# heyblackC/DFMIR

Hardware: AMD Instinct MI355X
Metric: train-step image-pairs/sec (fwd+bwd): 2D 256x256 bs=16 and 3D 160^3 bs=1 (higher is better)
Workload: dtype f32 (fp16x2-split MFMA, fp32 accumulate)

## Files before the change

### dfmir_amd/_lib.py

```python
import ctypes
import os
from ctypes import c_float, c_int, c_longlong, c_void_p, POINTER, Structure

_HERE = os.path.dirname(os.path.abspath(__file__))
LIB_PATH = os.environ.get("DFMIR_HIP_LIB") or os.path.join(_HERE, "libdfmir_hip.so")


class DfConvGeom(Structure):
    _fields_ = [(n, c_int) for n in (
        "N", "Cin", "Cout", "Di", "Hi", "Wi", "Do", "Ho", "Wo", "KD", "KH", "KW",
        "stride", "dil", "pd", "ph", "pw", "pad_mode", "act")] + [("slope", c_float)]


P = c_void_p
_GP = POINTER(DfConvGeom)
_SIGS = {
    "dfmir_abi_version": [],
    "dfmir_set_option": [ctypes.c_char_p, ctypes.c_char_p],
    "dfmir_get_option": [ctypes.c_char_p, ctypes.c_char_p, c_int],
    "dfmir_conv_fwd": [_GP, P, P, P, P, P],
    "dfmir_conv_wgrad": [_GP, P, P, P, P],
    "dfmir_bias_grad": [P, P, c_int, c_int, c_longlong, P],
    "dfmir_weight_pack": [P, P, c_int, c_int, c_int, c_int, P],
    "dfmir_weight_pack_floats": [c_int, c_int, c_int],
    "dfmir_weight_pack_batch": [P, c_int, P, c_int, P],
    "dfmir_conv3x3_res_ok": [_GP],
    "dfmir_conv3x3_fwd_scaled_res": [_GP, P, P, c_int, P, P, P, P, c_int, P, P],
    "dfmir_conv3x3_reflect_ring_ok": [_GP],
    "dfmir_conv3x3_reflect_ring_len": [_GP],
    "dfmir_conv3x3_reflect_ring": [_GP, P, P, P, c_int, P, P, P],
    "dfmir_conv_fwd_scaled": [_GP, P, P, c_int, P, P, P, P],
    "dfmir_conv_wgrad_scaled": [_GP, P, P, c_int, P, P, c_int, P, P, P],
    "dfmir_conv_wgrad_scaled_ch": [_GP, P, P, c_int, P, P, c_int, P, P, P, P],
    "dfmir_instnorm_bwd_pmax_ok": [c_longlong],
    "dfmir_instnorm_bwd_pmax": [P, P, P, P, P, c_int, c_longlong, c_int, P, P, c_int, P, P],
    "dfmir_patch_gather_bwd_gp": [P, P, P, c_int, c_int, c_longlong, c_int, c_int, P, P, P],
    "dfmir_patch_gather_bwd_any": [P, P, P, c_int, c_int, c_longlong, c_int, c_int, P, P, P],
    "dfmir_absmax": [P, c_longlong, P, P],
    "dfmir_conv3d_split_ok": [_GP],
    "dfmir_conv3d_split_ws_floats": [c_int, c_int],
    "dfmir_conv3d_split_fwd": [_GP, P, P, c_int, P, P, P, P, P, P],
    "dfmir_conv3d_split_fwd_sub": [_GP, P, P, c_int, P, P, P, P, P, c_int, P],
    "dfmir_conv3d_split_fwd_actgrad": [_GP, P, P, c_int, P, P, P, P, P, c_int, P, c_float, P],
    "dfmir_conv3d_up_ok": [c_int] * 6,
    "dfmir_conv3d_wsplit_batch": [P, c_int, P],
    "dfmir_conv3d_split_is_pair": [c_int],
    "dfmir_conv3d_march_ok": [_GP],
    "dfmir_conv3d_march_fwd": [_GP, P, P, c_int, P, P, P, P, P, c_float, P],
    "dfmir_conv3d_tiny_ok": [_GP],
    "dfmir_conv3d_tiny_fwd": [_GP, P, P, P, P, P, P, c_float, P],
    "dfmir_conv3d_s2c2_ok": [_GP],
    "dfmir_conv3d_s2c2_fwd": [_GP, P, P, P, P, P, P],
    "dfmir_conv3d_s2c2_wgrad": [_GP, P, P, P, P],
    "dfmir_conv3d_s2_ok": [_GP],
    "dfmir_conv3d_s2_fwd": [_GP, P, P, P, P, P, P],
    "dfmir_conv3d_s2_wgrad": [_GP, P, P, P, P, P],
    "dfmir_conv3d_s2_dgrad_ok": [_GP],
    "dfmir_conv3d_s2_dgrad": [_GP, P, P, P, P],
    "dfmir_conv3d_up_ws_floats": [c_int, c_int],
    "dfmir_conv3d_up_fwd": [P, P, c_int, P, c_int, P, P] + [c_int] * 6 + [P],
    "dfmir_conv3d_up_skip2_fwd": [P, P, c_int, P, P, c_int, c_int, P, P, P, P, P] + [c_int] * 7 + [c_float, P],
    "dfmir_conv3d_up_dgrad_ws_floats": [c_int, c_int],
    "dfmir_conv3d_up_dgrad": [P, P, c_int, P, c_int, P, P, P, P, c_float] + [c_int] * 6 + [P],
    "dfmir_conv3d_split_fwd_add": [_GP, P, P, c_int, P, c_int, c_int, P, P, P, P, P],
    "dfmir_conv3d_split_wgrad_ok": [_GP],
    "dfmir_conv3d_split_wgrad": [_GP, P, P, c_int, P, P, c_int, P, P],
# ... 95 lines not shown
    "dfmir_det_begin": [P, c_longlong, P, c_longlong, P, c_int, P, c_longlong, P, c_int, ctypes.c_double, P],
    "dfmir_det_end": [P, P, c_longlong, P, c_longlong, P],
    "dfmir_fill_zero": [P, c_longlong, P],
    "dfmir_sum_scaled": [P, P, c_longlong, c_float, P],
    "dfmir_fill_from_scalar": [P, P, c_longlong, c_float, P],
    "dfmir_adam_step": [P, P, P, P, c_longlong] + [c_float] * 7 + [P],
}

_lib = None


class DfmirHipError(RuntimeError):
    pass


def lib():
    global _lib
    if _lib is None:
        import torch
        if not os.path.exists(LIB_PATH):
            raise DfmirHipError(
                "libdfmir_hip.so not found at %s -- build it with `python -c 'import __graft_entry__ as g; "
                "g.build()'` or `make -C dfmir_amd/csrc` (there is no CPU fallback)" % LIB_PATH)
        h = ctypes.CDLL(LIB_PATH)
        for name, args in _SIGS.items():
            fn = getattr(h, name)
            fn.argtypes = args
            fn.restype = c_int
        h.dfmir_weight_pack_floats.restype = c_longlong
        h.dfmir_conv3d_split_ws_floats.restype = c_longlong
        h.dfmir_conv3d_up_ws_floats.restype = c_longlong
        h.dfmir_conv3d_up_dgrad_ws_floats.restype = c_longlong
        h.dfmir_conv3d_upwgrad_ws_floats.restype = c_longlong
        h.dfmir_flow_smooth_ws_floats.restype = c_longlong
        h.dfmir_nmi_ws_floats.restype = c_longlong
        h.dfmir_warp_dice_ws_floats.restype = c_longlong
        h.dfmir_label_hausdorff_ws_bytes.restype = c_longlong
        h.dfmir_dice_ws_floats.restype = c_longlong
        h.dfmir_mse_ws_floats.restype = c_longlong
        h.dfmir_warp_bwd_own_ws_floats.restype = c_longlong
        h.dfmir_resize_bwd_ws_floats.restype = c_longlong
        h.dfmir_last_error.argtypes = []
        h.dfmir_last_error.restype = ctypes.c_char_p
        _lib = h
    return _lib


def check(rc):
    if rc != 0:
        msg = lib().dfmir_last_error()
        raise DfmirHipError(msg.decode() if msg else "dfmir_hip error %d" % rc)


def set_option(name, value=None):
    check(lib().dfmir_set_option(name.encode(), None if value is None else str(value).encode()))


def get_option(name):
    buf = ctypes.create_string_buffer(256)
    n = lib().dfmir_get_option(name.encode(), buf, 256)
    return None if n < 0 else buf.value.decode()


def exported_symbols():
    return sorted(list(_SIGS.keys()) + ["dfmir_last_error"])
```

### dfmir_amd/csrc/conv.hip

```cpp
#include "conv3x3_common.h"
#include <stdlib.h>
#include <vector>

typedef float f32x16 __attribute__((ext_vector_type(16)));

struct ConvK {
  DfConvGeom g;
  int kc, nchunks;
  int Dm, Hm, Wm, ncx, ncy, ncz;
};

static inline void df_chunking(int Cin, int& kc, int& nchunks) {
  nchunks = (Cin + 15) / 16;
  int per = (Cin + nchunks - 1) / nchunks;
  kc = (per + 1) & ~1;
  if (kc < 2) kc = 2;
}

template <bool DIL2>
__device__ __forceinline__ bool conv_pixel(const ConvK& k, long long pp, long long P, int& n, int& oz, int& oy, int& ox,
                                           int& cls) {
  const DfConvGeom& g = k.g;
  cls = 0;
  if (pp >= P) { n = oz = oy = ox = 0; return false; }
// ... 611 lines not shown
    for (int r = ly; r < T * 32; r += 8) {
      const int t = r >> 5, ci = ci0 + (r & 31), co = co0 + lx;
      float v = 0.f;
      if (ci < Cin && co < Cout) {
        const long long j = ((long long)t * Cin + ci) * Cout + co;
        v = jb.src[j];
        jb.src[j] = 0.f;
      }
      tile[lx][(r & 31) * T + t] = v;
    }
    __syncthreads();
    const int ncol = 32 * T;
    for (int e = threadIdx.x; e < 32 * ncol; e += 256) {
      const int c = e / ncol, q = e - c * ncol;
      const int co = co0 + c, ci = ci0 + q / T;
      if (co < Cout && ci < Cin) jb.dst[((long long)co * Cin + ci0) * T + q] += tile[c][q];
    }
    __syncthreads();
  }
}

bool df_conv3x3_fwd_try(const DfConvGeom* g, const float* x, const float* w_tcc, const float* bias,
                        float* y, hipStream_t st, int* rc);
bool df_conv3x3_wgrad_try(const DfConvGeom* g, const float* x, const float* dy, float* dw_tcc,
                          hipStream_t st, int* rc);
bool df_conv3x3_small_wgrad_try(const DfConvGeom* g, const float* x, const float* dy, float* dw_tcc, hipStream_t st,
                                int* rc);
bool df_conv3x3_split_fwd_try(const DfConvGeom* g, const float* x, const float* x_amax, int x_n, const float* w_packed,
                              const float* bias, const float* res, const float* ring, int ring_rl, float* y,
                              hipStream_t st, int* rc);
int df_conv3x3_split_res_ok(const DfConvGeom* g);
bool df_conv3x3_split_wgrad_try(const DfConvGeom* g, const float* x, const float* x_amax, int x_n, const float* dy,
                                const float* dy_amax, int dy_n, float* dw_tcc, float* db, hipStream_t st, int* rc,
                                const float* dy_pmax);
int df_weight_split_launch(const float* w_tcc, float* packed, int K, int M, int npart, hipStream_t st);
float* df_weight_probe_slots(float* packed, int K, int M);
int df_absmax_launch(const float* x, long long n, float* out, hipStream_t st, bool zero_first);
bool df_conv3d_fwd_try(const DfConvGeom* g, const float* x, const float* w_tcc, const float* bias, float* y,
                       hipStream_t st, int* rc);
bool df_conv3d_wgrad_try(const DfConvGeom* g, const float* x, const float* dy, float* dw_tcc, hipStream_t st,
                         int* rc);
static bool use_generic_only() {
  static DfOptInt o{"DFMIR_CONV_GENERIC", 0};
  return o.get() == 1;
}

static int check_geom(const DfConvGeom* g) {
  if (!g) return -1;
  if (g->N <= 0 || g->Cin <= 0 || g->Cout <= 0) return -1;
  if (g->Di <= 0 || g->Hi <= 0 || g->Wi <= 0 || g->Do <= 0 || g->Ho <= 0 || g->Wo <= 0) return -1;
  if (g->KD <= 0 || g->KH <= 0 || g->KW <= 0 || g->KD > 15 || g->KH > 15 || g->KW > 15) return -1;
  if (g->stride < 1 || g->dil < 1) return -1;
  if (g->pad_mode != 0 && g->pad_mode != 1) return -1;
  if (g->pad_mode == 1 && g->dil != 1) return -1;
  return 0;
}

static int conv_fwd_impl(const DfConvGeom* g, const float* x, const float* x_amax, int x_n, const float* w_tcc,
                         const float* bias, float* y, void* stream);
extern "C" int dfmir_conv_fwd(const DfConvGeom* g, const float* x, const float* w_tcc,
                              const float* bias, float* y, void* stream) {
  return conv_fwd_impl(g, x, nullptr, 0, w_tcc, bias, y, stream);
}
extern "C" int dfmir_conv_fwd_scaled(const DfConvGeom* g, const float* x, const float* x_amax, int x_amax_n,
                                     const float* w_tcc, const float* bias, float* y, void* stream) {
  return conv_fwd_impl(g, x, x_amax, x_amax_n, w_tcc, bias, y, stream);
}
// ... 82 lines not shown
      } else {
        dim3 grid((unsigned)((Ps + 255) / 256), 1);
        if (g->Cout > 32) conv_mfma_k<1, 4, 2, 2, true><<<grid, 256, 0, st>>>(xs, w_tcc, bias, ys, k);
        else conv_mfma_k<1, 4, 1, 2, true><<<grid, 256, 0, st>>>(xs, w_tcc, bias, ys, k);
      }
    } else if (small_p && g->Cout <= 64) {
      dim3 grid((unsigned)((Ps + 63) / 64), (unsigned)((g->Cout + 63) / 64));
      conv_mfma_k<2, 2, 1, 1><<<grid, 256, 0, st>>>(xs, w_tcc, bias, ys, k);
    } else if (g->Cout > 64) {
      const long long big = ((Ps + 127) / 128) * ((g->Cout + 127) / 128);
      static DfOptInt big_o{"DFMIR_GEMM_BIG_MIN", 256};
  const int big_min = big_o.get();
      if (big < big_min) {
        dim3 grid((unsigned)((Ps + 63) / 64), (unsigned)((g->Cout + 63) / 64));
        conv_mfma_k<2, 2, 1, 1><<<grid, 256, 0, st>>>(xs, w_tcc, bias, ys, k);
      } else {
        dim3 grid((unsigned)((Ps + 127) / 128), (unsigned)((g->Cout + 127) / 128));
        conv_mfma_k<2, 2, 2, 2><<<grid, 256, 0, st>>>(xs, w_tcc, bias, ys, k);
      }
    } else if (g->Cout > 32) {
      dim3 grid((unsigned)((Ps + 255) / 256), 1);
      conv_mfma_k<1, 4, 2, 2><<<grid, 256, 0, st>>>(xs, w_tcc, bias, ys, k);
    } else {
      dim3 grid((unsigned)((Ps + 255) / 256), 1);
      conv_mfma_k<1, 4, 1, 2><<<grid, 256, 0, st>>>(xs, w_tcc, bias, ys, k);
    }
    DF_LAUNCH_CHECK();
  }
  return 0;
}

static int conv_wgrad_impl(const DfConvGeom* g, const float* x, const float* x_amax, int x_n, const float* dy,
                           const float* dy_amax, int dy_n, float* dw_tcc, float* db, void* stream,
                           const float* dy_pmax = nullptr);
extern "C" int dfmir_conv_wgrad_scaled_ch(const DfConvGeom* g, const float* x, const float* x_amax, int x_amax_n,
                                          const float* dy, const float* dy_amax, int dy_amax_n, const float* dy_pmax,
                                          float* dw_tcc, float* db, void* stream) {
  return conv_wgrad_impl(g, x, x_amax, x_amax_n, dy, dy_amax, dy_amax_n, dw_tcc, db, stream, dy_pmax);
}
extern "C" int dfmir_conv_wgrad(const DfConvGeom* g, const float* x, const float* dy, float* dw_tcc,
                                void* stream) {
  return conv_wgrad_impl(g, x, nullptr, 0, dy, nullptr, 0, dw_tcc, nullptr, stream);
}
extern "C" int dfmir_conv_wgrad_scaled(const DfConvGeom* g, const float* x, const float* x_amax, int x_amax_n,
                                       const float* dy, const float* dy_amax, int dy_amax_n, float* dw_tcc,
                                       float* db, void* stream) {
  return conv_wgrad_impl(g, x, x_amax, x_amax_n, dy, dy_amax, dy_amax_n, dw_tcc, db, stream);
}
static int bias_grad_launch(const float* dy, float* db, int N, int C, long long S, hipStream_t st);
static int conv_wgrad_impl(const DfConvGeom* g, const float* x, const float* x_amax, int x_n, const float* dy,
                           const float* dy_amax, int dy_n, float* dw_tcc, float* db, void* stream, const float* dy_pmax) {
  DF_ARG_CHECK(check_geom(g) == 0 && x && dy && dw_tcc);
  DF_ARG_CHECK(g->dil == 1 && g->Cin < (1 << 19));
  hipStream_t st = (hipStream_t)stream;
  if (!use_generic_only()) {
    int rc = 0;
    if (df_conv3x3_split_wgrad_try(g, x, x_amax, x_n, dy, dy_amax, dy_n, dw_tcc, db, st, &rc, dy_pmax)) return rc;
  }
  if (db) {
    const int rcb = bias_grad_launch(dy, db, g->N, g->Cout, (long long)g->Do * g->Ho * g->Wo, st);
    if (rcb) return rcb;
  }
  if (!use_generic_only()) {
    int rc = 0;
    if (df_conv3x3_wgrad_try(g, x, dy, dw_tcc, st, &rc)) return rc;
    if (df_conv3x3_small_wgrad_try(g, x, dy, dw_tcc, st, &rc)) return rc;
    if (df_conv3d_wgrad_try(g, x, dy, dw_tcc, st, &rc)) return rc;
  }
  {
    static DfOptFlag no1x1_o{"DFMIR_NO_1X1_WGRAD"};
    const long long S1 = (long long)g->Di * g->Hi * g->Wi;
    if (!use_generic_only() && !no1x1_o.get() && g->KD == 1 && g->KH == 1 && g->KW == 1 && g->stride == 1 && g->pd == 0 &&
        g->ph == 0 && g->pw == 0 && g->Do == g->Di && g->Ho == g->Hi && g->Wo == g->Wi && (S1 & 3) == 0 && S1 >= 64 &&
        ((reinterpret_cast<uintptr_t>(x) | reinterpret_cast<uintptr_t>(dy)) & 15) == 0 && g->Cin >= 8 && g->Cout >= 8) {
      const long long cpi = (S1 + 63) / 64, total = (long long)g->N * cpi;
      const unsigned ny = (unsigned)((g->Cin + 63) / 64), nz = (unsigned)((g->Cout + 63) / 64);
      long long want = 1024 / ((long long)ny * nz);
      if (want < 1) want = 1;
      long long maxs = (total + 7) / 8;
      if (maxs < 1) maxs = 1;
      if (want > maxs) want = maxs;
      const long long cpb = (total + want - 1) / want;
      const unsigned nx = (unsigned)((total + cpb - 1) / cpb);
      conv1x1_wgrad_k<<<dim3(nx, ny, nz), 256, 0, st>>>(x, dy, dw_tcc, g->N, g->Cin, g->Cout, S1, cpi, cpb, df_det_fx());
      DF_LAUNCH_CHECK();
      return 0;
    }
  }
  long long P = (long long)g->N * g->Do * g->Ho * g->Wo;
  const int J = g->KD * g->KH * g->KW * g->Cin;
// ... 141 lines not shown
```

### dfmir_amd/csrc/conv3x3s.hip

```cpp
#include "split_f16.h"

#ifndef PP_COMPUTE_PRIO
#define PP_COMPUTE_PRIO 1
#endif
#ifndef CS_COMPUTE_PRIO
#define CS_COMPUTE_PRIO 1
#endif
#ifndef CS_STORE_PRIO
#define CS_STORE_PRIO 0
#endif
typedef __bf16 bf16x8 __attribute__((ext_vector_type(8)));
typedef __bf16 bf16x2 __attribute__((ext_vector_type(2)));
typedef _Float16 f16x2 __attribute__((ext_vector_type(2)));
typedef float f32x2 __attribute__((ext_vector_type(2)));

__device__ __forceinline__ unsigned pk_bf16(float a, float b) {
  const f32x2 v = {a, b};
  return __builtin_bit_cast(unsigned, __builtin_convertvector(v, bf16x2));
}

template <int NSP>
__device__ __forceinline__ void split_pair(float x0, float x1, unsigned (&p)[NSP]) {
  if constexpr (NSP == 3) {
    p[0] = pk_bf16(x0, x1);
// ... 970 lines not shown
      conv3x3_split_cs_k<true, 32, 16><<<dim3((unsigned)nb, 1u), 512, 0, st>>>(x, ws, bias, y, kc, sc);
    }
    hipError_t e = hipGetLastError();
    *rc = (e == hipSuccess) ? 0 : df_set_error((int)e, __FILE__, __LINE__);
    return true;
  }
  if (res || ring) { *rc = df_set_error((int)hipErrorInvalidValue, __FILE__, __LINE__); return true; }
  k.tiles_per_img = (int)((HWo + 255) / 256);
  const bool big = g->Cout > 64;
  dim3 grid((unsigned)(g->N * k.tiles_per_img), big ? (unsigned)((g->Cout + 127) / 128) : 1u);
  if (mode == 2) {
    if (big) conv3x3_split_pp_k<2, 400, 128><<<grid, 512, 0, st>>>(x, ws, bias, y, k, sc);
    else conv3x3_split_pp_k<2, 400, 64><<<grid, 512, 0, st>>>(x, ws, bias, y, k, sc);
  } else {
    if (big) conv3x3_split_pp_k<3, 400, 128><<<grid, 512, 0, st>>>(x, ws, bias, y, k, sc);
    else conv3x3_split_pp_k<3, 400, 64><<<grid, 512, 0, st>>>(x, ws, bias, y, k, sc);
  }
  hipError_t e = hipGetLastError();
  *rc = (e == hipSuccess) ? 0 : df_set_error((int)e, __FILE__, __LINE__);
  return true;
}

struct WS3P {
  int N, Cin, Cout, H, W, pad_mode;
  int runs_per_row, runs_per_img, runs_total, runs_per_block;
  const float* x_amax;
  const float* dy_amax;
  int x_n, dy_n;
  float* db;
  const float* dy_pmax;
  int swap;
  float* dbx;
  const float* fx;
};

template <int NSP, int BC>
__global__ __launch_bounds__(512, 1) void conv3x3_wgrad_split_k(const float* __restrict__ x,
                                                                const float* __restrict__ dy,
                                                                float* __restrict__ dwt, WS3P k) {
  using P = Prod<NSP>;
  constexpr int CT = 64, NWC = BC / 32, KS = 4 / NWC, NSTEP = 18 / KS;
  constexpr int XSLAB = 2 * CT;
  __shared__ __attribute__((aligned(16))) u32x4 Xc[NSP * 3 * 4 * XSLAB];
  __shared__ __attribute__((aligned(16))) u32x4 Dy[NSP * 2 * 2 * BC];
  __shared__ float bsum[BC];

  const int tid = threadIdx.x, lane = tid & 63, wid = tid >> 6;
  const bool want_db = k.db != nullptr && blockIdx.y == 0;
  if (tid < BC) bsum[tid] = 0.f;
  float bacc = 0.f;
  const int wc = wid % NWC, wi = (wid / NWC) & 1, kh = wid / (2 * NWC);
  const int l31 = lane & 31, lhi = lane >> 5;
  const int HW = k.H * k.W;
  const int ci0 = blockIdx.y * CT, co0 = blockIdx.z * BC;
  const int run_beg = blockIdx.x * k.runs_per_block;
  int run_end = run_beg + k.runs_per_block;
  if (run_end > k.runs_total) run_end = k.runs_total;

  float xscale = 1.f, dscale = 1.f, oscale = 1.f, oscale2 = 1.f;
  if (NSP == 2) {
    __shared__ float red[17];
    const int ex = scale_exp(reduce_absmax(k.x_amax, k.x_n, red));
    __syncthreads();
    const int ed = scale_exp(reduce_absmax(k.dy_amax, k.dy_n, red));
    xscale = pow2f(ex); dscale = pow2f(ed); oscale = pow2f(-ex); oscale2 = pow2f(-ed);
  }
// ... 318 lines not shown
__global__ __launch_bounds__(512, 1) void conv3x3_wgrad_split2_k(const float* __restrict__ x,
                                                                 const float* __restrict__ dy,
                                                                 float* __restrict__ dwt, WS3P k) {
  constexpr int NSP = 2, BC = 128, CT = 64;
  using P = Prod<2>;
#ifndef W2_CTPAD
#define W2_CTPAD 0
#endif
  constexpr int CTP = CT + W2_CTPAD;
  constexpr int XSLAB = 2 * CTP;
  constexpr int XCU = NSP * 3 * 4 * XSLAB, DYU = NSP * 2 * 2 * BC;
  __shared__ __attribute__((aligned(16))) u32x4 Xc[2 * XCU];
  __shared__ __attribute__((aligned(16))) u32x4 Dy[2 * DYU];
  __shared__ float bsum[BC];
  __shared__ float red[17];

  const int tid = threadIdx.x, lane = tid & 63;
  const int wid = __builtin_amdgcn_readfirstlane((int)(threadIdx.x >> 6));
  const bool want_db = k.db != nullptr && blockIdx.y == 0;
  if (tid < BC) bsum[tid] = 0.f;
  float bacc = 0.f, baccx = 0.f;
  const int wc = wid & 3, wi = wid >> 2;
  const int l31 = lane & 31, lhi = lane >> 5;
  const int HW = k.H * k.W;
  const int ci0 = blockIdx.y * CT, co0 = blockIdx.z * BC;
  const int run_beg = blockIdx.x * k.runs_per_block;
  int run_end = run_beg + k.runs_per_block;
  if (run_end > k.runs_total) run_end = k.runs_total;

  const int ex = scale_exp(reduce_absmax(k.x_amax, k.x_n, red));
  __syncthreads();
  const int ed = scale_exp(reduce_absmax(k.dy_amax, k.dy_n, red));
  __shared__ int edc[BC];
  if (tid < BC) {
    int e = ed;
    if (k.dy_pmax) {
      float m = 0.f;
      if (co0 + tid < k.Cout)
        for (int n = 0; n < k.N; ++n) m = fmaxf(m, k.dy_pmax[(long long)n * k.Cout + co0 + tid]);
      e = scale_exp(m);
    }
    edc[tid] = e;
  }
  __syncthreads();

  const int xc = tid & 63, xu = (tid >> 6) & 1, xr = tid >> 7;
  const int dc = tid & (BC - 1), du = (tid >> 7) & 1, dk = tid >> 8;
  const bool xin = k.dbx != nullptr && blockIdx.z == 0 && (xr == 1 || xr == 2);
  const float xscale = pow2f(ex), dscale = pow2f(edc[dc]), oscale = pow2f(-ex), oscale2 = pow2f(-edc[wc * 32 + l31]);
  const unsigned hw4 = (unsigned)HW * 4u;
  constexpr unsigned OOB = 0x80000000u;

  f32x16 acc[9];
#pragma unroll
  for (int t = 0; t < 9; ++t)
#pragma unroll
    for (int r = 0; r < 16; ++r) acc[t][r] = 0.f;

  u32x4 rxa, rxb, rda, rdb;
  unsigned rxl, rxr;

#ifndef W2_KO
#define W2_KO 0
#endif
#define W2_GLOAD(run_)                                                                           \
  if (!(W2_KO & 1) || k.N < 0) {                                                                 \
    const bool live_ = (run_) < run_end;                                                         \
    const int n_ = live_ ? (run_) / k.runs_per_img : 0;                                          \
    const int q_ = live_ ? (run_) - n_ * k.runs_per_img : 0;                                     \
    const int yp_ = q_ / k.runs_per_row, xs_ = q_ - yp_ * k.runs_per_row;                        \
    const int y0_ = 2 * yp_, x0_ = 16 * xs_ + 8 * xu;                                            \
    const __amdgpu_buffer_rsrc_t bx_ = __builtin_amdgcn_make_buffer_rsrc(                        \
        const_cast<float*>(x + (long long)n_ * k.Cin * HW), 0, live_ ? (unsigned)(k.Cin * HW) * 4u : 0u, 0x00020000); \
    const __amdgpu_buffer_rsrc_t bd_ = __builtin_amdgcn_make_buffer_rsrc(                        \
        const_cast<float*>(dy + (long long)n_ * k.Cout * HW), 0, live_ ? (unsigned)(k.Cout * HW) * 4u : 0u, 0x00020000); \
    const bool cok_ = ci0 + xc < k.Cin;                                                          \
// ... 124 lines not shown
    for (int run = run_beg; run < run_end; ++run) {
      const int buf = (run - run_beg) & 1;
      W2T(0)
      W2_PRIO(W2_PRIO_G1);
      if (!(W2_KO & 8) || k.N < 0) W2_MMA_PHASE(buf);
      __builtin_amdgcn_sched_barrier(0);
      W2T(1)
      W2_PRIO(W2_PRIO_C);
      W2T_VM()
      W2_LSTORE(buf ^ 1);
      W2_GLOAD(run + 2);
      W2T(2)
      __syncthreads();
      W2T(3)
    }
  }
#undef W2_GLOAD
#undef W2_LSTORE
#undef W2_LOADA
#undef W2_MMA_PHASE
#undef W2_UDX
#undef W2_UROW

  if (want_db) {
    atomicAdd(&bsum[dc], bacc);
    __syncthreads();
    if (tid < BC && co0 + tid < k.Cout) atomicAdd(&k.db[co0 + tid], bsum[tid]);
  }
  if (k.dbx != nullptr && blockIdx.z == 0) {
    atomicAdd(&bsum[xc], baccx);
    __syncthreads();
    if (tid < CT && ci0 + tid < k.Cin) atomicAdd(&k.dbx[ci0 + tid], bsum[tid]);
  }
  if (k.swap) {
    __syncthreads();
    float* T = reinterpret_cast<float*>(Xc) + wid * (32 * 33);
#pragma unroll
    for (int t = 0; t < 9; ++t) {
#pragma unroll
      for (int r = 0; r < 16; ++r) T[(4 * lhi + (r & 3) + 8 * (r >> 2)) * 33 + l31] = acc[t][r] * oscale * oscale2;
      __syncthreads();
      const int ci = ci0 + wi * 32 + l31;
#pragma unroll
      for (int r = 0; r < 16; ++r) {
        const int col = 4 * lhi + (r & 3) + 8 * (r >> 2);
        const int co = co0 + wc * 32 + col;
        const float v = T[l31 * 33 + col];
        if (ci < k.Cin && co < k.Cout) df_acc(dwt, ((long long)(8 - t) * k.Cout + co) * k.Cin + ci, v, k.fx);
      }
      __syncthreads();
    }
    return;
  }
  const int co = co0 + wc * 32 + l31;
  if (co < k.Cout) {
#pragma unroll
    for (int t = 0; t < 9; ++t) {
#pragma unroll
      for (int r = 0; r < 16; ++r) {
        const int ci = ci0 + wi * 32 + 4 * lhi + (r & 3) + 8 * (r >> 2);
        if (ci < k.Cin) df_acc(dwt, ((long long)t * k.Cin + ci) * k.Cout + co, acc[t][r] * oscale * oscale2, k.fx);
      }
    }
  }
}

bool df_conv3x3_split_wgrad_swaps(const DfConvGeom* g) {
  static DfOptFlag ns_o{"DFMIR_WGRAD_NO_SWAP"}, v1_o{"DFMIR_WGRAD_V1"};
  const bool off = ns_o.get() || v1_o.get();
  return !off && df_split_mode() == 2 && g->KD == 1 && g->KH == 3 && g->KW == 3 && g->Di == 1 && g->Do == 1 && g->stride == 1 &&
         g->dil == 1 && g->ph == 1 && g->pw == 1 && g->pd == 0 && g->Ho == g->Hi && g->Wo == g->Wi && g->pad_mode == 0 &&
         g->Cout == 64 && g->Cin > 64;
}
bool df_conv3x3_split_wgrad_try(const DfConvGeom* g, const float* x, const float* x_amax, int x_n, const float* dy,
                                const float* dy_amax, int dy_n, float* dw_tcc, float* db, hipStream_t st, int* rc,
                                const float* dy_pmax) {
  const int mode = df_split_mode();
  if (mode == 0 || (mode == 2 && !(x_amax && dy_amax && x_n > 0 && dy_n > 0))) return false;
  if (!(g->KD == 1 && g->KH == 3 && g->KW == 3 && g->Di == 1 && g->Do == 1 && g->stride == 1 && g->dil == 1))
    return false;
  if (g->ph != 1 || g->pw != 1 || g->pd != 0 || g->Ho != g->Hi || g->Wo != g->Wi) return false;
  if (g->Cout < 64 || g->Cin < 64) return false;
  const bool wide = g->Cout > 64;
  if ((g->Hi & 1) || (g->Wi & 15) || g->Hi < 2) return false;
  const long long HW = (long long)g->Hi * g->Wi;
  if (HW * g->Cin * 4 >= (1LL << 31) || HW * g->Cout * 4 >= (1LL << 31)) return false;
  const bool swap = mode == 2 && x_amax && dy_amax && df_conv3x3_split_wgrad_swaps(g);
  WS3P k{g->N, g->Cin, g->Cout, g->Hi, g->Wi, g->pad_mode, g->Wi / 16, 0, 0, 0, x_amax, dy_amax, x_n, dy_n, db, dy_pmax, 0, nullptr, df_det_fx()};
  if (swap) {
    k.Cin = g->Cout; k.Cout = g->Cin;
    k.x_amax = dy_amax; k.dy_amax = x_amax; k.x_n = dy_n; k.dy_n = x_n;
    k.db = nullptr; k.dbx = db; k.dy_pmax = nullptr; k.swap = 1;
  }
  k.runs_per_img = (g->Hi / 2) * k.runs_per_row;
  const long long total = (long long)g->N * k.runs_per_img;
  if (total >= (1LL << 30)) return false;
  k.runs_total = (int)total;
  const unsigned ny = (k.Cin + 63) / 64, nz = (wide || swap) ? (k.Cout + 127) / 128 : 1;
  long long want = 256 / ((long long)ny * nz);
  if (want < 1) want = 1;
  long long maxs = (k.runs_total + 7) / 8;
  if (maxs < 1) maxs = 1;
  if (want > maxs) want = maxs;
  k.runs_per_block = (int)((k.runs_total + want - 1) / want);
  const unsigned nx = (k.runs_total + k.runs_per_block - 1) / k.runs_per_block;
  const dim3 grid(nx, ny, nz);
  if (mode == 2) {
    static DfOptFlag v1_o{"DFMIR_WGRAD_V1"};
    const bool v1 = v1_o.get();
    if (swap) conv3x3_wgrad_split2_k<<<grid, 512, 0, st>>>(dy, x, dw_tcc, k);
    else if (wide && !v1) conv3x3_wgrad_split2_k<<<grid, 512, 0, st>>>(x, dy, dw_tcc, k);
    else if (wide) conv3x3_wgrad_split_k<2, 128><<<grid, 512, 0, st>>>(x, dy, dw_tcc, k);
    else conv3x3_wgrad_split_k<2, 64><<<grid, 512, 0, st>>>(x, dy, dw_tcc, k);
  } else {
    if (wide) conv3x3_wgrad_split_k<3, 128><<<grid, 512, 0, st>>>(x, dy, dw_tcc, k);
    else conv3x3_wgrad_split_k<3, 64><<<grid, 512, 0, st>>>(x, dy, dw_tcc, k);
  }
  hipError_t e = hipGetLastError();
  *rc = (e == hipSuccess) ? 0 : df_set_error((int)e, __FILE__, __LINE__);
  return true;
}
```

### dfmir_amd/ops.py

```python
import ctypes
import os

import numpy as np
import torch
from torch.autograd import Function
from torch.autograd.function import once_differentiable

from ._lib import DfConvGeom, DfmirHipError, check, lib

_VP = ctypes.c_void_p


def _p(t):
    return None if t is None else _VP(t.data_ptr())


def _st():
    return _VP(torch.cuda.current_stream().cuda_stream)


def _need(*ts):
    for t in ts:
        if t is None:
            continue
# ... 264 lines not shown
                prof(kind, flops * cu / Cout, launch, 3.0 * pad_k * pad_m * flops * cu / Cout)
            else:
                prof(kind, flops * cu / Cout, launch)
        else:
            prof(kind, flops, launch)
    return y


_LAST_ACTGRAD = [False]
_NO_TINY3D = _env_on("DFMIR_CONV3D_NO_TINY")
_NO_TINYVOL = _env_on("DFMIR_NO_TINYVOL")
_NO_S2 = _env_on("DFMIR_CONV3D_NO_S2")
_NO_FLOW_MARCH = _env_on("DFMIR_CONV3D_NO_FLOW_MARCH")
_NO_ACTGRAD = _env_on("DFMIR_NO_ACTGRAD")


def _tag_ok(t, tag):
    return tag is not None and tag[-2] == t._version and tag[-1] == t.data_ptr()


_UPWGRAD_MIN_VOX = int(os.environ.get("DFMIR_UPWGRAD_MIN_VOX", "400000"))
_UPWGRAD_MIN_VOX_FUSED = 50000
_UPWGRAD_WS = {}


def _upwgrad_ws(device):
    key = (device.index, torch.cuda.current_stream(device).cuda_stream)
    ws = _UPWGRAD_WS.get(key)
    if ws is None:
        ws = _UPWGRAD_WS[key] = torch.zeros(int(lib().dfmir_conv3d_upwgrad_ws_floats()), device=device)
    return ws


_DET = {"on": _env_on("DFMIR_DETERMINISTIC_WGRAD")}


def set_deterministic_wgrad(on):
    _DET["on"] = bool(on)


def deterministic_wgrad():
    return _DET["on"]


class _DetAcc(object):
    def __init__(self, n_dw, n_db, count, x, x_amax, dy, dy_amax):
        head = int(lib().dfmir_det_head_floats())
        self.n_dw, self.n_db = int(n_dw), int(n_db)
        self.scr = torch.empty(head + 2 * (self.n_dw + self.n_db), device=dy.device, dtype=torch.float32)
        check(lib().dfmir_det_begin(_p(self.scr), self.n_dw + self.n_db, _p(x), 0 if x is None else x.numel(), _p(x_amax),
                                    0 if x_amax is None else x_amax.numel(), _p(dy), dy.numel(), _p(dy_amax),
                                    0 if dy_amax is None else dy_amax.numel(), float(count), _st()))
        self.dw = self.scr[head:head + 2 * self.n_dw]
        self.db = self.scr[head + 2 * self.n_dw:] if self.n_db else None

    def end(self, dw_out, db_out):
        check(lib().dfmir_det_end(_p(self.scr), _p(dw_out), self.n_dw, _p(db_out), self.n_db if db_out is not None else 0, _st()))

    def abort(self):
        check(lib().dfmir_det_end(_p(self.scr), None, 0, None, 0, _st()))


def bias_grad(dy5, db):
    N, C = dy5.shape[0], dy5.shape[1]
    S = dy5.numel() // (N * C)
    if not _DET["on"]:
# ... 41 lines not shown
            and bool(lib().dfmir_conv3d_s2c2_ok(ctypes.byref(g))))
    s2m = (parts is None and not s2c2 and tuple(K) == (3, 3, 3) and stride == 2 and not _NO_S2
           and bool(lib().dfmir_conv3d_s2_ok(ctypes.byref(g))))
    det = _DetAcc(dw.numel(), Cout if db is not None else 0, N * Do * Ho * Wo, x5 if parts is None else None, x_amax,
                  dy5, dy_amax) if _DET["on"] else None
    dw_real, db_real = dw, db
    if det is not None:
        dw, db = det.dw, None

    def launch():
        if s2c2:
            if db is not None:
                check(lib().dfmir_bias_grad(_p(dy5), _p(db), dy5.shape[0], Cout, Do * Ho * Wo, _st()))
            check(lib().dfmir_conv3d_s2c2_wgrad(ctypes.byref(g), _p(x5), _p(dy5), _p(dw), _st()))
            return
        if s2m:
            check(lib().dfmir_conv3d_s2_wgrad(ctypes.byref(g), _p(x5), _p(dy5), _p(dw), _p(db), _st()))
            return
        if parts is not None:
            if upw:
                check(lib().dfmir_conv3d_upwgrad(ctypes.byref(g), _p(parts[0]), _p(parts[1]), parts[0].shape[1],
                                                 _p(x_amax), x_amax.numel(), _p(dy5), _p(dy_amax), dy_amax.numel(),
                                                 _p(dw), _p(db), _p(_upwgrad_ws(dy5.device)), _st()))
                return
            check(lib().dfmir_conv3d_split_wgrad_upcat(ctypes.byref(g), _p(parts[0]), _p(parts[1]), parts[0].shape[1],
                                                       _p(x_amax), x_amax.numel(), _p(dy5), _p(dy_amax), dy_amax.numel(),
                                                       _p(dw), _p(db), _st()))
            return
        if split3d:
            check(lib().dfmir_conv3d_split_wgrad_db(ctypes.byref(g), _p(x5), _p(x_amax), x_amax.numel(), _p(dy5),
                                                    _p(dy_amax), dy_amax.numel(), _p(dw), _p(db), _st()))
            return
        pm = dy_pmax if (dy_pmax is not None and dy_pmax.numel() == N * Cout and dy_amax is not None) else None
        check(lib().dfmir_conv_wgrad_scaled_ch(ctypes.byref(g), _p(x5), _p(x_amax),
                                               0 if x_amax is None else x_amax.numel(), _p(dy5), _p(dy_amax),
                                               0 if dy_amax is None else dy_amax.numel(), _p(pm), _p(dw), _p(db), _st()))

    if det is not None:
        try:
            launch()
            if db_real is not None:
                check(lib().dfmir_bias_grad(_p(dy5), _p(det.db), dy5.shape[0], Cout, Do * Ho * Wo, _st()))
        except BaseException:
            det.abort()
            raise
        det.end(dw_real, db_real)
        return dw_real
    prof = _CONV_PROFILER[0]
    if prof is None:
        launch()
    else:
        is3x3 = (tuple(K) == (1, 3, 3) and stride == 1 and Di == 1 and pad[1] == 1 and pad[2] == 1
                 and Cout >= 64 and Cin >= 32 and (Hi * Wi) % 32 == 0 and Wi % 32 == 0)
        size = "L" if Cout > 64 else ("M" if Cout > 32 else "S")
        is3d = (tuple(K) == (3, 3, 3) and stride == 1 and tuple(pad) == (1, 1, 1) and pad_mode == 0 and Cout <= 32
                and Wi % 4 == 0)
        flops = 2.0 * N * Cout * Do * Ho * Wo * Cin * T
        kind = ("wgrad3dt_S" if (s2c2 or s2m) else
                ("wgrad3x3_" if is3x3 else (("wgrad3ds_" if split3d else "wgrad3d_") if is3d else "conv_wgrad_")) + size)
        if split3d and is3d and not s2c2 and getattr(prof, "accepts_issued", False):
            if upw:
                Ca_, Cb_ = parts[0].shape[1], parts[1].shape[1]
                skip_ = (64.0 / 54.0) if Cb_ == 2 else (28.0 / 27.0) * (8.0 * ((Cb_ + 7) // 8)) / Cb_
                pad_ = ((8.0 / 27.0) * Ca_ + skip_ * Cb_) / Cin * (32.0 / Cout)
                kind = "wgrad3dup_" + size
            elif Cout < 8:
                pad_ = (28.0 / 27.0) * (8.0 / Cout) * (32.0 / Cin)
            elif parts is None and lib().dfmir_conv3d_wgrad_is_march_at(ctypes.byref(g), _p(x5), _p(dy5)):
                pad_ = 28.0 / 27.0
# ... 2105 lines not shown
```

### include/dfmir_hip.h

```cpp
#ifndef DFMIR_HIP_H
#define DFMIR_HIP_H

#ifdef __cplusplus
extern "C" {
#endif

#define DFMIR_ABI_VERSION 14

int dfmir_abi_version(void);
const char* dfmir_last_error(void);

int dfmir_set_option(const char* name, const char* value);
int dfmir_get_option(const char* name, char* buf, int buf_len);

typedef struct DfConvGeom {
  int N, Cin, Cout;
  int Di, Hi, Wi;
  int Do, Ho, Wo;
  int KD, KH, KW;
  int stride, dil;
  int pd, ph, pw;
  int pad_mode;
  int act;
  float slope;
// ... 41 lines not shown
                              int b_amax_n, int Cb, const float* w_tcc, float* ws, const float* bias, float* y,
                              float* y_amax, int N, int Ca, int Cout, int D, int H, int W, int act, float slope,
                              void* stream);
long long dfmir_conv3d_up_dgrad_ws_floats(int Ca, int Cout);
int dfmir_conv3d_up_dgrad(const float* dy, const float* dy_amax, int dy_amax_n, const float* w_tcc, int Ktot, float* ws,
                          float* da, float* da_amax, const float* act_src, float act_slope, int N, int Ca, int Cout, int D,
                          int H, int W, void* stream);
int dfmir_conv3d_split_fwd_add(const DfConvGeom* g, const float* b, const float* b_amax, int b_amax_n, const float* w_tcc,
                               int Ktot, int koff, float* ws, const float* bias, float* y, float* y_amax, void* stream);
int dfmir_conv3d_split_wgrad_ok(const DfConvGeom* g);
int dfmir_conv3d_split_wgrad(const DfConvGeom* g, const float* x, const float* x_amax, int x_amax_n, const float* dy,
                             const float* dy_amax, int dy_amax_n, float* dw_tcc, void* stream);
int dfmir_conv3d_split_wgrad_upcat(const DfConvGeom* g, const float* a, const float* b, int Ca, const float* x_amax,
                                   int x_amax_n, const float* dy, const float* dy_amax, int dy_amax_n, float* dw_tcc,
                                   float* db, void* stream);
int dfmir_conv3d_upwgrad_ok(const DfConvGeom* g, int Ca);
long long dfmir_conv3d_upwgrad_ws_floats(void);
int dfmir_conv3d_upwgrad(const DfConvGeom* g, const float* a, const float* b, int Ca, const float* x_amax, int x_amax_n,
                         const float* dy, const float* dy_amax, int dy_amax_n, float* dw_tcc, float* db, float* ws,
                         void* stream);
int dfmir_conv3d_split_wgrad_db(const DfConvGeom* g, const float* x, const float* x_amax, int x_amax_n, const float* dy,
                                const float* dy_amax, int dy_amax_n, float* dw_tcc, float* db, void* stream);
int dfmir_conv3d_wgrad_is_march(const DfConvGeom* g);
int dfmir_conv3d_wgrad_is_march_at(const DfConvGeom* g, const float* x, const float* dy);
int dfmir_probe_merge(const float* a, const float* b, float* out, void* stream);
int dfmir_conv_wgrad(const DfConvGeom* g, const float* x, const float* dy, float* dw_tcc,
                     void* stream);
int dfmir_conv_wgrad_scaled(const DfConvGeom* g, const float* x, const float* x_amax, int x_amax_n,
                            const float* dy, const float* dy_amax, int dy_amax_n, float* dw_tcc, float* db,
                            void* stream);
int dfmir_conv_wgrad_scaled_ch(const DfConvGeom* g, const float* x, const float* x_amax, int x_amax_n, const float* dy,
                               const float* dy_amax, int dy_amax_n, const float* dy_pmax, float* dw_tcc, float* db,
                               void* stream);
int dfmir_bias_grad(const float* dy, float* db, int N, int C, long long S, void* stream);
long long dfmir_weight_pack_floats(int Cout, int Cin, int T);
int dfmir_weight_pack(const float* w, float* w_tcc, int Cout, int Cin, int T, int mode, void* stream);
int dfmir_weight_unpack(const float* g_tcc, float* g, int Cout, int Cin, int T, void* stream);
int dfmir_conv3x3_res_ok(const DfConvGeom* g);
int dfmir_conv3x3_fwd_scaled_res(const DfConvGeom* g, const float* x, const float* x_amax, int x_amax_n,
                                 const float* w_tcc, const float* bias, const float* res, const float* ring,
                                 int ring_len, float* y, void* stream);

int dfmir_conv3x3_reflect_ring_ok(const DfConvGeom* g);
int dfmir_conv3x3_reflect_ring_len(const DfConvGeom* g);
int dfmir_conv3x3_reflect_ring(const DfConvGeom* g, const float* dy, const float* dy_cols, const float* dy_amax,
                               int dy_amax_n, const float* wd_packed, float* ring, void* stream);

typedef struct DfPackJob {
  const float* w;
  float* packed;
  int Cout, Cin, T, mode;
} DfPackJob;
int dfmir_weight_pack_batch(const DfPackJob* jobs, int njobs, void* table_dev, int upload, void* stream);

typedef struct DfUnpackJob {
  float* src;
  float* dst;
  int Cout, Cin, T, reserved;
} DfUnpackJob;
int dfmir_weight_unpack_add_batch(const DfUnpackJob* jobs, int njobs, long long max_total, void* stream);

int dfmir_conv7x7_c1_fwd(const float* x, const float* w, const float* bias, float* y, int N, int H, int W, int Cout,
                         int pad_mode, void* stream);
int dfmir_conv7x7_c1_wgrad(const float* x, const float* dy, float* dw, float* db, int N, int H, int W, int Cout,
                           int pad_mode, void* stream);

// ... 188 lines not shown
```

Before: 213.0.

## Replace atomic wgrad accumulation with per-block partials plus a reduce kernel

```diff
diff --git a/dfmir_amd/_lib.py b/dfmir_amd/_lib.py
--- a/dfmir_amd/_lib.py
+++ b/dfmir_amd/_lib.py
@@ -32,6 +32,8 @@
     "dfmir_conv_fwd_scaled": [_GP, P, P, c_int, P, P, P, P],
     "dfmir_conv_wgrad_scaled": [_GP, P, P, c_int, P, P, c_int, P, P, P],
     "dfmir_conv_wgrad_scaled_ch": [_GP, P, P, c_int, P, P, c_int, P, P, P, P],
+    "dfmir_conv_wgrad_scaled_ch_ws": [_GP, P, P, c_int, P, P, c_int, P, P, P, P, c_longlong, P],
+    "dfmir_conv3x3_wgrad_ws_floats": [_GP],
     "dfmir_instnorm_bwd_pmax_ok": [c_longlong],
     "dfmir_instnorm_bwd_pmax": [P, P, P, P, P, c_int, c_longlong, c_int, P, P, c_int, P, P],
     "dfmir_patch_gather_bwd_gp": [P, P, P, c_int, c_int, c_longlong, c_int, c_int, P, P, P],
@@ -193,6 +195,7 @@
         h.dfmir_conv3d_up_ws_floats.restype = c_longlong
         h.dfmir_conv3d_up_dgrad_ws_floats.restype = c_longlong
         h.dfmir_conv3d_upwgrad_ws_floats.restype = c_longlong
+        h.dfmir_conv3x3_wgrad_ws_floats.restype = c_longlong
         h.dfmir_flow_smooth_ws_floats.restype = c_longlong
         h.dfmir_nmi_ws_floats.restype = c_longlong
         h.dfmir_warp_dice_ws_floats.restype = c_longlong
diff --git a/dfmir_amd/csrc/conv.hip b/dfmir_amd/csrc/conv.hip
--- a/dfmir_amd/csrc/conv.hip
+++ b/dfmir_amd/csrc/conv.hip
@@ -667,7 +667,7 @@
 int df_conv3x3_split_res_ok(const DfConvGeom* g);
 bool df_conv3x3_split_wgrad_try(const DfConvGeom* g, const float* x, const float* x_amax, int x_n, const float* dy,
                                 const float* dy_amax, int dy_n, float* dw_tcc, float* db, hipStream_t st, int* rc,
-                                const float* dy_pmax);
+                                const float* dy_pmax, float* ws = nullptr, long long ws_floats = 0);
 int df_weight_split_launch(const float* w_tcc, float* packed, int K, int M, int npart, hipStream_t st);
 float* df_weight_probe_slots(float* packed, int K, int M);
 int df_absmax_launch(const float* x, long long n, float* out, hipStream_t st, bool zero_first);
@@ -816,7 +816,12 @@
 
 static int conv_wgrad_impl(const DfConvGeom* g, const float* x, const float* x_amax, int x_n, const float* dy,
                            const float* dy_amax, int dy_n, float* dw_tcc, float* db, void* stream,
-                           const float* dy_pmax = nullptr);
+                           const float* dy_pmax = nullptr, float* ws = nullptr, long long ws_floats = 0);
+extern "C" int dfmir_conv_wgrad_scaled_ch_ws(const DfConvGeom* g, const float* x, const float* x_amax, int x_amax_n,
+                                             const float* dy, const float* dy_amax, int dy_amax_n, const float* dy_pmax,
+                                             float* dw_tcc, float* db, float* ws, long long ws_floats, void* stream) {
+  return conv_wgrad_impl(g, x, x_amax, x_amax_n, dy, dy_amax, dy_amax_n, dw_tcc, db, stream, dy_pmax, ws, ws_floats);
+}
 extern "C" int dfmir_conv_wgrad_scaled_ch(const DfConvGeom* g, const float* x, const float* x_amax, int x_amax_n,
                                           const float* dy, const float* dy_amax, int dy_amax_n, const float* dy_pmax,
                                           float* dw_tcc, float* db, void* stream) {
@@ -833,13 +838,14 @@
 }
 static int bias_grad_launch(const float* dy, float* db, int N, int C, long long S, hipStream_t st);
 static int conv_wgrad_impl(const DfConvGeom* g, const float* x, const float* x_amax, int x_n, const float* dy,
-                           const float* dy_amax, int dy_n, float* dw_tcc, float* db, void* stream, const float* dy_pmax) {
+                           const float* dy_amax, int dy_n, float* dw_tcc, float* db, void* stream, const float* dy_pmax,
+                           float* ws, long long ws_floats) {
   DF_ARG_CHECK(check_geom(g) == 0 && x && dy && dw_tcc);
   DF_ARG_CHECK(g->dil == 1 && g->Cin < (1 << 19));
   hipStream_t st = (hipStream_t)stream;
   if (!use_generic_only()) {
     int rc = 0;
-    if (df_conv3x3_split_wgrad_try(g, x, x_amax, x_n, dy, dy_amax, dy_n, dw_tcc, db, st, &rc, dy_pmax)) return rc;
+    if (df_conv3x3_split_wgrad_try(g, x, x_amax, x_n, dy, dy_amax, dy_n, dw_tcc, db, st, &rc, dy_pmax, ws, ws_floats)) return rc;
   }
   if (db) {
     const int rcb = bias_grad_launch(dy, db, g->N, g->Cout, (long long)g->Do * g->Ho * g->Wo, st);
diff --git a/dfmir_amd/csrc/conv3x3s.hip b/dfmir_amd/csrc/conv3x3s.hip
--- a/dfmir_amd/csrc/conv3x3s.hip
+++ b/dfmir_amd/csrc/conv3x3s.hip
@@ -1026,6 +1026,7 @@
   int swap;
   float* dbx;
   const float* fx;
+  float* part;
 };
 
 template <int NSP, int BC>
@@ -1410,16 +1411,25 @@
   __syncthreads();
   const int ed = scale_exp(reduce_absmax(k.dy_amax, k.dy_n, red));
   __shared__ int edc[BC];
-  if (tid < BC) {
-    int e = ed;
-    if (k.dy_pmax) {
-      float m = 0.f;
-      if (co0 + tid < k.Cout)
-        for (int n = 0; n < k.N; ++n) m = fmaxf(m, k.dy_pmax[(long long)n * k.Cout + co0 + tid]);
-      e = scale_exp(m);
-    }
-    edc[tid] = e;
-  }
+  __shared__ float pmx[4][BC];
+  if (k.dy_pmax) {
+    const int c = tid & (BC - 1), q = tid >> 7;
+    float m0 = 0.f, m1 = 0.f, m2 = 0.f, m3 = 0.f;
+    if (co0 + c < k.Cout) {
+      const float* p = k.dy_pmax + co0 + c;
+      int n = q;
+      for (; n + 12 < k.N; n += 16) {
+        const float v0 = p[(long long)n * k.Cout], v1 = p[(long long)(n + 4) * k.Cout];
+        const float v2 = p[(long long)(n + 8) * k.Cout], v3 = p[(long long)(n + 12) * k.Cout];
+        m0 = fmaxf(m0, v0); m1 = fmaxf(m1, v1); m2 = fmaxf(m2, v2); m3 = fmaxf(m3, v3);
+      }
+      for (; n < k.N; n += 4) m0 = fmaxf(m0, p[(long long)n * k.Cout]);
+    }
+    pmx[q][c] = fmaxf(fmaxf(m0, m1), fmaxf(m2, m3));
+    __syncthreads();
+  }
+  if (tid < BC)
+    edc[tid] = k.dy_pmax ? scale_exp(fmaxf(fmaxf(pmx[0][tid], pmx[1][tid]), fmaxf(pmx[2][tid], pmx[3][tid]))) : ed;
   __syncthreads();
 
   const int xc = tid & 63, xu = (tid >> 6) & 1, xr = tid >> 7;
@@ -1610,6 +1620,15 @@
     __syncthreads();
     if (tid < CT && ci0 + tid < k.Cin) atomicAdd(&k.dbx[ci0 + tid], bsum[tid]);
   }
+  if (k.part) {
+    float* pt = k.part + (((long long)blockIdx.x * gridDim.y + blockIdx.y) * gridDim.z + blockIdx.z) * (9 * CT * BC) +
+                (wi * 32 + 4 * lhi) * BC + wc * 32 + l31;
+#pragma unroll
+    for (int t = 0; t < 9; ++t)
+#pragma unroll
+      for (int r = 0; r < 16; ++r) pt[(t * CT + (r & 3) + 8 * (r >> 2)) * BC] = acc[t][r] * oscale * oscale2;
+    return;
+  }
   if (k.swap) {
     __syncthreads();
     float* T = reinterpret_cast<float*>(Xc) + wid * (32 * 33);
@@ -1650,39 +1669,122 @@
          g->dil == 1 && g->ph == 1 && g->pw == 1 && g->pd == 0 && g->Ho == g->Hi && g->Wo == g->Wi && g->pad_mode == 0 &&
          g->Cout == 64 && g->Cin > 64;
 }
-bool df_conv3x3_split_wgrad_try(const DfConvGeom* g, const float* x, const float* x_amax, int x_n, const float* dy,
-                                const float* dy_amax, int dy_n, float* dw_tcc, float* db, hipStream_t st, int* rc,
-                                const float* dy_pmax) {
-  const int mode = df_split_mode();
-  if (mode == 0 || (mode == 2 && !(x_amax && dy_amax && x_n > 0 && dy_n > 0))) return false;
+
+__global__ __launch_bounds__(256) void conv3x3_wgrad_reduce_k(const float* __restrict__ part, float* __restrict__ dwt,
+                                                              int Cin, int Cout, int nx, int swap) {
+  constexpr int TILE = 9 * 64 * 128;
+  __shared__ f32x4 sm[3][64];
+  const int o = threadIdx.x & 63;
+  const int q = __builtin_amdgcn_readfirstlane((int)(threadIdx.x >> 6));
+  const int e = (blockIdx.x * 64 + o) * 4;
+  const long long sstride = (long long)gridDim.y * gridDim.z * TILE;
+  const int chunk = (nx + 3) >> 2;
+  int s = q * chunk;
+  const int s1 = s + chunk < nx ? s + chunk : nx;
+  const float* p = part + ((long long)blockIdx.y * gridDim.z + blockIdx.z) * TILE + e + s * sstride;
+  f32x4 a = {0.f, 0.f, 0.f, 0.f};
+  for (; s + 8 <= s1; s += 8, p += 8 * sstride) {
+    f32x4 v[8];
+#pragma unroll
+    for (int i = 0; i < 8; ++i) v[i] = *reinterpret_cast<const f32x4*>(p + i * sstride);
+#pragma unroll
+    for (int i = 0; i < 8; ++i) a += v[i];
+  }
+  for (; s < s1; ++s, p += sstride) a += *reinterpret_cast<const f32x4*>(p);
+  if (q) sm[q - 1][o] = a;
+  __syncthreads();
+  if (q) return;
+  a = ((a + sm[0][o]) + sm[1][o]) + sm[2][o];
+  const int t = e >> 13, row = (e >> 7) & 63, col = e & 127;
+  const int ci = blockIdx.y * 64 + row, co = blockIdx.z * 128 + col;
+  if (ci >= Cin || co >= Cout) return;
+  if (swap) {
+#pragma unroll
+    for (int i = 0; i < 4; ++i)
+      if (co + i < Cout) dwt[((long long)(8 - t) * Cout + co + i) * Cin + ci] += a[i];
+    return;
+  }
+  float* d = dwt + ((long long)t * Cin + ci) * Cout + co;
+  if ((Cout & 3) == 0 && (reinterpret_cast<uintptr_t>(dwt) & 15) == 0) {
+    f32x4* d4 = reinterpret_cast<f32x4*>(d);
+    *d4 = *d4 + a;
+  } else {
+#pragma unroll
+    for (int i = 0; i < 4; ++i)
+      if (co + i < Cout) d[i] += a[i];
+  }
+}
+
+struct W3Plan {
+  bool wide, swap;
+  int Cin, Cout;
+  int runs_per_row, runs_per_img, runs_total, runs_per_block;
+  unsigned nx, ny, nz;
+};
+static bool split_wgrad_plan(const DfConvGeom* g, int mode, W3Plan* p) {
   if (!(g->KD == 1 && g->KH == 3 && g->KW == 3 && g->Di == 1 && g->Do == 1 && g->stride == 1 && g->dil == 1))
     return false;
   if (g->ph != 1 || g->pw != 1 || g->pd != 0 || g->Ho != g->Hi || g->Wo != g->Wi) return false;
   if (g->Cout < 64 || g->Cin < 64) return false;
-  const bool wide = g->Cout > 64;
   if ((g->Hi & 1) || (g->Wi & 15) || g->Hi < 2) return false;
   const long long HW = (long long)g->Hi * g->Wi;
   if (HW * g->Cin * 4 >= (1LL << 31) || HW * g->Cout * 4 >= (1LL << 31)) return false;
-  const bool swap = mode == 2 && x_amax && dy_amax && df_conv3x3_split_wgrad_swaps(g);
-  WS3P k{g->N, g->Cin, g->Cout, g->Hi, g->Wi, g->pad_mode, g->Wi / 16, 0, 0, 0, x_amax, dy_amax, x_n, dy_n, db, dy_pmax, 0, nullptr, df_det_fx()};
+  p->wide = g->Cout > 64;
+  p->swap = mode == 2 && df_conv3x3_split_wgrad_swaps(g);
+  p->Cin = p->swap ? g->Cout : g->Cin;
+  p->Cout = p->swap ? g->Cin : g->Cout;
+  p->runs_per_row = g->Wi / 16;
+  p->runs_per_img = (g->Hi / 2) * p->runs_per_row;
+  const long long total = (long long)g->N * p->runs_per_img;
+  if (total >= (1LL << 30)) return false;
+  p->runs_total = (int)total;
+  p->ny = (p->Cin + 63) / 64;
+  p->nz = (p->wide || p->swap) ? (p->Cout + 127) / 128 : 1;
+  long long want = 256 / ((long long)p->ny * p->nz);
+  if (want < 1) want = 1;
+  long long maxs = (p->runs_total + 7) / 8;
+  if (maxs < 1) maxs = 1;
+  if (want > maxs) want = maxs;
+  p->runs_per_block = (int)((p->runs_total + want - 1) / want);
+  p->nx = (p->runs_total + p->runs_per_block - 1) / p->runs_per_block;
+  return true;
+}
+static bool split_wgrad_partials(int mode, const W3Plan& p) {
+  static DfOptFlag v1_o{"DFMIR_WGRAD_V1"};
+  static DfOptFlag at_o{"DFMIR_WGRAD_ATOMIC_TAIL"};
+  return mode == 2 && (p.swap || (p.wide && !v1_o.get())) && !at_o.get();
+}
+extern "C" long long dfmir_conv3x3_wgrad_ws_floats(const DfConvGeom* g) {
+  if (!g) return 0;
+  const int mode = df_split_mode();
+  W3Plan p;
+  if (!split_wgrad_plan(g, mode, &p) || !split_wgrad_partials(mode, p)) return 0;
+  return (long long)p.nx * p.ny * p.nz * (9 * 64 * 128);
+}
+bool df_conv3x3_split_wgrad_try(const DfConvGeom* g, const float* x, const float* x_amax, int x_n, const float* dy,
+                                const float* dy_amax, int dy_n, float* dw_tcc, float* db, hipStream_t st, int* rc,
+                                const float* dy_pmax, float* ws, long long ws_floats) {
+  const int mode = df_split_mode();
+  if (mode == 0 || (mode == 2 && !(x_amax && dy_amax && x_n > 0 && dy_n > 0))) return false;
+  W3Plan p;
+  if (!split_wgrad_plan(g, mode, &p)) return false;
+  const bool wide = p.wide, swap = p.swap;
+  WS3P k{g->N, g->Cin, g->Cout, g->Hi, g->Wi, g->pad_mode, p.runs_per_row, p.runs_per_img, p.runs_total, p.runs_per_block,
+         x_amax, dy_amax, x_n, dy_n, db, dy_pmax, 0, nullptr, df_det_fx(), nullptr};
   if (swap) {
     k.Cin = g->Cout; k.Cout = g->Cin;
     k.x_amax = dy_amax; k.dy_amax = x_amax; k.x_n = dy_n; k.dy_n = x_n;
     k.db = nullptr; k.dbx = db; k.dy_pmax = nullptr; k.swap = 1;
   }
-  k.runs_per_img = (g->Hi / 2) * k.runs_per_row;
-  const long long total = (long long)g->N * k.runs_per_img;
-  if (total >= (1LL << 30)) return false;
-  k.runs_total = (int)total;
-  const unsigned ny = (k.Cin + 63) / 64, nz = (wide || swap) ? (k.Cout + 127) / 128 : 1;
-  long long want = 256 / ((long long)ny * nz);
-  if (want < 1) want = 1;
-  long long maxs = (k.runs_total + 7) / 8;
-  if (maxs < 1) maxs = 1;
-  if (want > maxs) want = maxs;
-  k.runs_per_block = (int)((k.runs_total + want - 1) / want);
-  const unsigned nx = (k.runs_total + k.runs_per_block - 1) / k.runs_per_block;
-  const dim3 grid(nx, ny, nz);
+  const dim3 grid(p.nx, p.ny, p.nz);
+  const long long need = (long long)p.nx * p.ny * p.nz * (9 * 64 * 128);
+  if (ws && !k.fx && split_wgrad_partials(mode, p)) {
+    if (ws_floats < need || (reinterpret_cast<uintptr_t>(ws) & 15)) {
+      *rc = df_set_error(-1, __FILE__, __LINE__);
+      return true;
+    }
+    k.part = ws;
+  }
   if (mode == 2) {
     static DfOptFlag v1_o{"DFMIR_WGRAD_V1"};
     const bool v1 = v1_o.get();
@@ -1690,6 +1792,8 @@
     else if (wide && !v1) conv3x3_wgrad_split2_k<<<grid, 512, 0, st>>>(x, dy, dw_tcc, k);
     else if (wide) conv3x3_wgrad_split_k<2, 128><<<grid, 512, 0, st>>>(x, dy, dw_tcc, k);
     else conv3x3_wgrad_split_k<2, 64><<<grid, 512, 0, st>>>(x, dy, dw_tcc, k);
+    if (k.part)
+      conv3x3_wgrad_reduce_k<<<dim3(9 * 64 * 128 / 256, p.ny, p.nz), 256, 0, st>>>(k.part, dw_tcc, k.Cin, k.Cout, (int)p.nx, k.swap);
   } else {
     if (wide) conv3x3_wgrad_split_k<3, 128><<<grid, 512, 0, st>>>(x, dy, dw_tcc, k);
     else conv3x3_wgrad_split_k<3, 64><<<grid, 512, 0, st>>>(x, dy, dw_tcc, k);
diff --git a/dfmir_amd/ops.py b/dfmir_amd/ops.py
--- a/dfmir_amd/ops.py
+++ b/dfmir_amd/ops.py
@@ -320,6 +320,20 @@
     return ws
 
 
+_WGRAD_WS = {}
+_WGRAD_WS_MIN = 256 * 73728
+
+
+def _wgrad_ws(device, need):
+    key = (device.index, torch.cuda.current_stream(device).cuda_stream)
+    ws = _WGRAD_WS.get(key)
+    if ws is None or ws.numel() < need:
+        if torch.cuda.is_current_stream_capturing():
+            return None
+        ws = _WGRAD_WS[key] = torch.empty(max(int(need), _WGRAD_WS_MIN), device=device, dtype=torch.float32)
+    return ws
+
+
 _DET = {"on": _env_on("DFMIR_DETERMINISTIC_WGRAD")}
 
 
@@ -427,9 +441,15 @@
                                                     _p(dy_amax), dy_amax.numel(), _p(dw), _p(db), _st()))
             return
         pm = dy_pmax if (dy_pmax is not None and dy_pmax.numel() == N * Cout and dy_amax is not None) else None
-        check(lib().dfmir_conv_wgrad_scaled_ch(ctypes.byref(g), _p(x5), _p(x_amax),
-                                               0 if x_amax is None else x_amax.numel(), _p(dy5), _p(dy_amax),
-                                               0 if dy_amax is None else dy_amax.numel(), _p(pm), _p(dw), _p(db), _st()))
+        ws = None
+        if det is None and x_amax is not None and dy_amax is not None:
+            need = int(lib().dfmir_conv3x3_wgrad_ws_floats(ctypes.byref(g)))
+            if need:
+                ws = _wgrad_ws(dy5.device, need)
+        check(lib().dfmir_conv_wgrad_scaled_ch_ws(ctypes.byref(g), _p(x5), _p(x_amax),
+                                                  0 if x_amax is None else x_amax.numel(), _p(dy5), _p(dy_amax),
+                                                  0 if dy_amax is None else dy_amax.numel(), _p(pm), _p(dw), _p(db),
+                                                  _p(ws), 0 if ws is None else ws.numel(), _st()))
 
     if det is not None:
         try:
diff --git a/include/dfmir_hip.h b/include/dfmir_hip.h
--- a/include/dfmir_hip.h
+++ b/include/dfmir_hip.h
@@ -97,6 +97,10 @@
 int dfmir_conv_wgrad_scaled_ch(const DfConvGeom* g, const float* x, const float* x_amax, int x_amax_n, const float* dy,
                                const float* dy_amax, int dy_amax_n, const float* dy_pmax, float* dw_tcc, float* db,
                                void* stream);
+long long dfmir_conv3x3_wgrad_ws_floats(const DfConvGeom* g);
+int dfmir_conv_wgrad_scaled_ch_ws(const DfConvGeom* g, const float* x, const float* x_amax, int x_amax_n, const float* dy,
+                                  const float* dy_amax, int dy_amax_n, const float* dy_pmax, float* dw_tcc, float* db,
+                                  float* ws, long long ws_floats, void* stream);
 int dfmir_bias_grad(const float* dy, float* db, int N, int C, long long S, void* stream);
 long long dfmir_weight_pack_floats(int Cout, int Cin, int T);
 int dfmir_weight_pack(const float* w, float* w_tcc, int Cout, int Cin, int T, int mode, void* stream);
```

New measurement: 214.3, median of 6. No clear change (+0.6%).
